# victorramirez952/tomography_3d_reconstructor

Hardware: AMD Instinct MI355X
Metric: Mvoxels/s (SDF+MC) on 1024^3 ellipsoid stack; achieved HBM GB/s vs peak (higher is better)
Workload: dtype f64

## Files before the change

### include/tomo_hip.h

```cpp
#ifndef TOMO_HIP_H
#define TOMO_HIP_H

#include <stddef.h>
#include <stdint.h>

#ifdef __cplusplus
extern "C" {
#endif

#define TOMO_OK 0
#define TOMO_E_ARG (-1)
#define TOMO_E_LAUNCH (-2)
#define TOMO_E_SIZE (-3)
#define TOMO_E_WORKSPACE (-4)

int tomo_abi_version(void);
const char *tomo_error_string(int code);
int tomo_host_mc_cell(const float *h_v, double iso, int8_t *h_tris, int *h_uses_centre);
double tomo_host_mc_edge_offset(double va, double vb);
void tomo_host_mc_centre_offset(const double *h_v8, double *h_out3);

int tomo_host_checksum(const void *h_data, int64_t nbytes, int nthreads, uint64_t *h_out);
int tomo_host_checksum_impl(const void *h_data, int64_t nbytes, int nthreads, int impl, uint64_t *h_out);
int64_t tomo_host_checksum_chunk_bytes(void);
// ... 61 lines not shown
int tomo_field_signs(const float *field, int Nz, int Ny, int Nx, int64_t pitch, int xorg, double iso, int z_begin,
                     int z_end, unsigned long long *signs, uint8_t *gcls, void *stream);

int tomo_mc_classify(const unsigned long long *signs, const uint8_t *gcls, int Nz, int Ny, int Nx, int xorg,
                     unsigned long long *seg_act, uint32_t *seg_cnt, void *stream);
int tomo_mc_scan_segments(const uint32_t *seg_cnt, int64_t nseg, uint32_t *seg_aoff, unsigned long long *totals,
                          void *workspace, int64_t workspace_bytes, void *stream);
int64_t tomo_mc_scan_workspace_bytes(int64_t n);
int tomo_mc_scan(const uint32_t *counts, int64_t n, uint32_t *off_a, uint32_t *off_b, uint32_t *nz_ids,
                 unsigned long long *totals, void *workspace, int64_t workspace_bytes, void *stream);
int tomo_mc_list(int Nz, int Ny, int Nx, int xorg, const uint32_t *seg_aoff, const unsigned long long *seg_act,
                 unsigned long long *vox_key, void *stream);
int tomo_mc_eval(const float *field, int Nz, int Ny, int Nx, int64_t pitch, int xorg, double iso,
                 const unsigned long long *vox_key, int64_t na, uint32_t *vox_counts, uint8_t *vox_flags, void *stream);
int tomo_mc_list_capped(int Nz, int Ny, int Nx, int xorg, const uint32_t *seg_aoff, const unsigned long long *seg_act,
                        unsigned long long *vox_key, int64_t cap, void *stream);
int tomo_mc_eval_capped(const float *field, int Nz, int Ny, int Nx, int64_t pitch, int xorg, double iso,
                        const unsigned long long *vox_key, int64_t cap, const unsigned long long *na_dev,
                        uint32_t *vox_counts, uint8_t *vox_flags, void *stream);
int tomo_mc_emit(const float *field, int Nz, int Ny, int Nx, int64_t pitch, int xorg, double iso,
                 const unsigned long long *vox_key, int64_t na, const unsigned long long *seg_act,
                 const uint32_t *seg_aoff, const uint32_t *vox_voff, const uint32_t *vox_foff, const uint8_t *vox_flags,
                 int z_offset, unsigned long long *vkey, float *vpos, int32_t *faces, unsigned long long *totals,
                 void *stream);

int tomo_mc_first_touch(const float *field, int Nz, int Ny, int Nx, int64_t pitch, int xorg, double iso,
                        const unsigned long long *vox_key, int64_t na, const unsigned long long *seg_act,
                        const uint32_t *seg_aoff, const uint32_t *vox_voff, const uint8_t *vox_flags, int mode,
                        uint32_t *created, const uint32_t *base, int32_t *ft_rank, unsigned long long *totals, void *stream);

int tomo_mc3_list(int Nz, int Ny, int Nx, int xorg, const uint32_t *seg_cnt, const unsigned long long *seg_act,
                  uint32_t *seg_blk, uint32_t *seg_aoff, unsigned long long *vox_key, int64_t cap, unsigned long long *tot,
                  void *stream);
int tomo_mc3_eval(const float *field, int Nz, int Ny, int Nx, int64_t pitch, int xorg, double iso,
                  const unsigned long long *vox_key, int64_t cap, const unsigned long long *tot, int z_offset,
                  uint32_t *vox_loc, int32_t *vox_til, uint8_t *vox_flags, uint16_t *vox_used, float *vox_f3, float *vox_c3,
                  uint32_t *blk3, void *stream);
int64_t tomo_mc3_slice_table_words(int Nz, int Ny);
int64_t tomo_mc3_sort_segments(int Nz, int Ny);
int tomo_mc3_scan(int Nz, int Ny, int Nx, int xorg, const uint32_t *seg_aoff, const uint32_t *vox_loc, int64_t cap,
                  uint32_t *blk3, uint32_t *slice_tab, unsigned long long *tot, int64_t cap_v, int64_t cap_f, void *stream);
int tomo_mc3_vertices(int Nz, int Ny, int Nx, int xorg, const unsigned long long *vox_key, int64_t cap,
                      const unsigned long long *tot, const uint32_t *vox_loc, const uint8_t *vox_flags, const float *vox_f3,
                      const float *vox_c3, const uint32_t *blk3, const uint32_t *slice_tab, int z_offset, int shift,
                      const double *cum, int64_t ncum, const double *adj, int64_t nadj, float mm_y, float mm_x, float *vrec,
                      uint32_t *keys, uint32_t *idx, void *stream);
int64_t tomo_mc3_sort_workspace_bytes(int64_t cap_v, int64_t nseg);
int tomo_mc3_sort_rank_top(const float *vrec, uint32_t *keys, uint32_t *idx, int64_t cap_v, int Nz, int Ny, const uint32_t *slice_tab,
                           unsigned long long *tot, float *uniq, int32_t *table, void *workspace, int64_t workspace_bytes,
                           float z_top, void *stream);
int tomo_mc3_sort_rank_fused(const float *vrec, const uint32_t *keys, int64_t cap_v, int Nz, int Ny, uint32_t *slice_tab,
                             unsigned long long *tot, float *uniq, int32_t *table, float z_top, void *stream);
int tomo_mc3_faces(int Nz, int Ny, int Nx, int xorg, const unsigned long long *vox_key, int64_t cap, unsigned long long *tot,
                   const unsigned long long *seg_act, const uint32_t *seg_aoff, const uint32_t *vox_loc, const int32_t *vox_til,
                   const uint16_t *vox_used, const uint32_t *blk3, const int32_t *table, int64_t *faces, int64_t cap_f,
                   void *stream);

int tomo_vertex_finalize(float *vpos, int64_t nv, int shift, const double *cum, int64_t ncum,
                         const double *adj, int64_t nadj, float mm_y, float mm_x, void *stream);
int64_t tomo_mesh_unique_workspace_bytes(int64_t nv);
int tomo_mesh_unique(const float *vpos, int64_t nv, float *uniq, int32_t *rank, unsigned long long *totals,
                     void *workspace, int64_t workspace_bytes, void *stream);
int tomo_mesh_lookup(const float *uniq, int64_t nu, const float *query, int64_t nq, int32_t *out,
                     unsigned long long *missing, void *stream);
int tomo_slab_top_rows(const float *uniq, const unsigned long long *tot, int64_t cap_v, int64_t cap, float *msg, void *stream);
int tomo_slab_lookup(const float *uniq, const unsigned long long *tot, int64_t cap_v, const float *msg, int64_t cap,
// ... 42 lines not shown
```

### tomography_3d_reconstructor_amd/_lib.py

```python
import ctypes
import os
import subprocess

_HERE = os.path.dirname(os.path.abspath(__file__))
SO_PATH = os.environ.get("TOMO_LIB") or os.path.join(_HERE, "libtomo_hip.so")
CSRC = os.path.join(_HERE, "csrc")

_c_i = ctypes.c_int
_c_i64 = ctypes.c_int64
_c_p = ctypes.c_void_p
_c_d = ctypes.c_double
_c_f = ctypes.c_float

SIGNATURES = {
    "tomo_abi_version": (_c_i, []),
    "tomo_error_string": (ctypes.c_char_p, [_c_i]),
    "tomo_host_mc_cell": (_c_i, [_c_p, _c_d, _c_p, _c_p]),
    "tomo_host_mc_edge_offset": (_c_d, [_c_d, _c_d]),
    "tomo_host_mc_centre_offset": (None, [_c_p, _c_p]),
    "tomo_host_checksum": (_c_i, [_c_p, _c_i64, _c_i, _c_p]),
    "tomo_host_checksum_impl": (_c_i, [_c_p, _c_i64, _c_i, _c_i, _c_p]),
    "tomo_host_checksum_chunk_bytes": (_c_i64, []),
    "tomo_host_checksum_part": (_c_i, [_c_p, _c_i64, _c_i64, _c_i, _c_i, _c_p]),
    "tomo_host_checksum_fold": (_c_i, [_c_p, _c_i64, _c_i64, _c_p]),
# ... 27 lines not shown
    "tomo_pack_close_ends": (_c_i, [_c_p, _c_p, _c_i, _c_i, _c_i, _c_p, _c_p]),
    "tomo_pack_bits_pair": (_c_i, [_c_p, _c_p, _c_i, _c_p, _c_p, _c_i, _c_i, _c_i, _c_p]),
    "tomo_slab_edges": (_c_i, [_c_p, _c_p, _c_i, _c_i, _c_i, _c_i, _c_p, _c_p, _c_i, _c_i, _c_p, _c_p, _c_p, _c_i, _c_p, _c_p, _c_p, _c_p,
                               _c_i, _c_p, _c_p]),
    "tomo_pack_close_range": (_c_i, [_c_p, _c_p, _c_i, _c_i, _c_i, _c_i, _c_i, _c_p, _c_p, _c_i, _c_i, _c_p]),
    "tomo_close_ends_workspace_words": (_c_i64, [_c_i, _c_i, _c_i]),
    "tomo_close_ends_scan": (_c_i, [_c_p, _c_i, _c_i, _c_i, _c_p, _c_p]),
    "tomo_close_ends_gp": (_c_i, [_c_p, _c_i, _c_i, _c_i, _c_p, _c_p, _c_p]),
    "tomo_morph_pass": (_c_i, [_c_p, _c_p, _c_i, _c_i, _c_i, _c_i, _c_p]),
    "tomo_morph_fused": (_c_i, [_c_p, _c_p, _c_i, _c_i, _c_i, ctypes.c_uint32, _c_i, _c_p]),
    "tomo_smooth": (_c_i, [_c_p, _c_p, _c_i, _c_i, _c_i, _c_i, _c_i, _c_p]),
    "tomo_extend_bits": (_c_i, [_c_p, _c_p, _c_i, _c_i, _c_i, _c_i, _c_p]),
    "tomo_field_fill": (_c_i, [_c_p, _c_p, _c_i, _c_i, _c_i, _c_i, _c_i, _c_p, _c_p, _c_p]),
    "tomo_field_fill_bits": (_c_i, [_c_p, _c_p, _c_i, _c_i, _c_i, _c_i, _c_p, _c_p, _c_p]),
    "tomo_field_span_bytes": (_c_i64, [_c_i, _c_i, _c_i, _c_i]),
    "tomo_field_fill_bits_sparse": (_c_i, [_c_p, _c_p, _c_i, _c_i, _c_i, _c_i, _c_p, _c_p, _c_p, _c_p]),
    "tomo_sign_rows": (_c_i64, [_c_i]),
    "tomo_field_signs_fused": (_c_i, [_c_i]),
    "tomo_sign_buffer_words": (_c_i64, [_c_i, _c_i, _c_i, _c_i]),
    "tomo_field_signs": (_c_i, [_c_p, _c_i, _c_i, _c_i, _c_i64, _c_i, _c_d, _c_i, _c_i, _c_p, _c_p, _c_p]),
    "tomo_mc_classify": (_c_i, [_c_p, _c_p, _c_i, _c_i, _c_i, _c_i, _c_p, _c_p, _c_p]),
    "tomo_mc_scan_segments": (_c_i, [_c_p, _c_i64, _c_p, _c_p, _c_p, _c_i64, _c_p]),
    "tomo_mc_scan_workspace_bytes": (_c_i64, [_c_i64]),
    "tomo_mc_scan": (_c_i, [_c_p, _c_i64, _c_p, _c_p, _c_p, _c_p, _c_p, _c_i64, _c_p]),
    "tomo_mc_list": (_c_i, [_c_i, _c_i, _c_i, _c_i, _c_p, _c_p, _c_p, _c_p]),
    "tomo_mc_eval": (_c_i, [_c_p, _c_i, _c_i, _c_i, _c_i64, _c_i, _c_d, _c_p, _c_i64, _c_p, _c_p, _c_p]),
    "tomo_mc_list_capped": (_c_i, [_c_i, _c_i, _c_i, _c_i, _c_p, _c_p, _c_p, _c_i64, _c_p]),
    "tomo_mc_eval_capped": (_c_i, [_c_p, _c_i, _c_i, _c_i, _c_i64, _c_i, _c_d, _c_p, _c_i64, _c_p, _c_p, _c_p, _c_p]),
    "tomo_mc_emit": (_c_i, [_c_p, _c_i, _c_i, _c_i, _c_i64, _c_i, _c_d, _c_p, _c_i64, _c_p, _c_p, _c_p, _c_p, _c_p, _c_i, _c_p,
                            _c_p, _c_p, _c_p, _c_p]),
    "tomo_mc_first_touch": (_c_i, [_c_p, _c_i, _c_i, _c_i, _c_i64, _c_i, _c_d, _c_p, _c_i64, _c_p, _c_p, _c_p, _c_p, _c_i, _c_p,
                                   _c_p, _c_p, _c_p, _c_p]),
    "tomo_mc3_list": (_c_i, [_c_i, _c_i, _c_i, _c_i, _c_p, _c_p, _c_p, _c_p, _c_p, _c_i64, _c_p, _c_p]),
    "tomo_mc3_eval": (_c_i, [_c_p, _c_i, _c_i, _c_i, _c_i64, _c_i, _c_d, _c_p, _c_i64, _c_p, _c_i, _c_p, _c_p, _c_p, _c_p, _c_p,
                             _c_p, _c_p, _c_p]),
    "tomo_mc3_slice_table_words": (_c_i64, [_c_i, _c_i]),
    "tomo_mc3_sort_segments": (_c_i64, [_c_i, _c_i]),
    "tomo_mc3_scan": (_c_i, [_c_i, _c_i, _c_i, _c_i, _c_p, _c_p, _c_i64, _c_p, _c_p, _c_p, _c_i64, _c_i64, _c_p]),
    "tomo_mc3_vertices": (_c_i, [_c_i, _c_i, _c_i, _c_i, _c_p, _c_i64, _c_p, _c_p, _c_p, _c_p, _c_p, _c_p, _c_p, _c_i, _c_i,
                                 _c_p, _c_i64, _c_p, _c_i64, _c_f, _c_f, _c_p, _c_p, _c_p, _c_p]),
    "tomo_mc3_sort_workspace_bytes": (_c_i64, [_c_i64, _c_i64]),
    "tomo_mc3_sort_rank_top": (_c_i, [_c_p, _c_p, _c_p, _c_i64, _c_i, _c_i, _c_p, _c_p, _c_p, _c_p, _c_p, _c_i64, _c_f, _c_p]),
    "tomo_mc3_sort_rank_fused": (_c_i, [_c_p, _c_p, _c_i64, _c_i, _c_i, _c_p, _c_p, _c_p, _c_p, _c_f, _c_p]),
    "tomo_mc3_faces": (_c_i, [_c_i, _c_i, _c_i, _c_i, _c_p, _c_i64, _c_p, _c_p, _c_p, _c_p, _c_p, _c_p, _c_p, _c_p, _c_p, _c_i64, _c_p]),
    "tomo_vertex_finalize": (_c_i, [_c_p, _c_i64, _c_i, _c_p, _c_i64, _c_p, _c_i64, _c_f, _c_f, _c_p]),
    "tomo_mesh_unique_workspace_bytes": (_c_i64, [_c_i64]),
    "tomo_mesh_unique": (_c_i, [_c_p, _c_i64, _c_p, _c_p, _c_p, _c_p, _c_i64, _c_p]),
    "tomo_mesh_lookup": (_c_i, [_c_p, _c_i64, _c_p, _c_i64, _c_p, _c_p, _c_p]),
    "tomo_slab_top_rows": (_c_i, [_c_p, _c_p, _c_i64, _c_i64, _c_p, _c_p]),
    "tomo_slab_lookup": (_c_i, [_c_p, _c_p, _c_i64, _c_p, _c_i64, _c_p, _c_p, _c_p]),
    "tomo_slab_summary": (_c_i, [_c_p, _c_i64, _c_p, _c_p, _c_i64, _c_i64, _c_p, _c_p]),
    "tomo_slab_lookup_summary": (_c_i, [_c_p, _c_p, _c_i64, _c_p, _c_i64, _c_p, _c_i64, _c_i64, _c_p, _c_p, _c_p]),
    "tomo_mc3_faces_slab": (_c_i, [_c_i, _c_i, _c_i, _c_i, _c_p, _c_i64, _c_p, _c_p, _c_p, _c_p, _c_p, _c_p, _c_p, _c_p, _c_p, _c_i64,
                                   _c_p, _c_i, _c_i, _c_p, _c_i64, _c_i64, _c_p]),
    "tomo_mesh_volume_area": (_c_i, [_c_p, _c_p, _c_i64, _c_p, _c_p]),
    "tomo_layer_colors": (_c_i, [_c_p, _c_i, _c_i64, _c_i64, _c_d, _c_d, _c_i, _c_d, _c_d, _c_i, _c_p, _c_p]),
    "tomo_mesh_edge_table_bytes": (_c_i64, [_c_i64]),
    "tomo_mesh_edges": (_c_i, [_c_p, _c_i64, _c_i64, _c_p, _c_i64, _c_p, _c_p]),
    "tomo_mesh_seam_edges": (_c_i, [_c_p, _c_i64, _c_i64, _c_i64, _c_p, _c_i64, _c_p, _c_p]),
    "tomo_mesh_seam_merge": (_c_i, [_c_p, _c_i64, _c_i64, _c_p, _c_i64, _c_p, _c_p]),
    "tomo_mesh_orient_workspace_bytes": (_c_i64, [_c_i64]),
    "tomo_mesh_orient": (_c_i, [_c_p, _c_i64, _c_i64, _c_p, _c_i64, _c_p, _c_p, _c_p]),
    "tomo_mesh_signed_volume": (_c_i, [_c_p, _c_p, _c_i64, _c_p, _c_p, _c_p]),
    "tomo_glb_pack_faces": (_c_i, [_c_p, _c_i64, _c_p, _c_p, _c_p, _c_i, _c_p]),
    "tomo_glb_pack_positions": (_c_i, [_c_p, _c_i, _c_i64, _c_p, _c_p, _c_p]),
    "tomo_mesh_vertex_normals_workspace_bytes": (_c_i64, [_c_i64, _c_i64]),
# ... 49 lines not shown
```

### tomography_3d_reconstructor_amd/csrc/mc.hip

```cpp
#include <cstring>
#include <cstdlib>
#include "tomo_common.h"
#include <rocprim/rocprim.hpp>

#define MC_LUT_QUAL __device__ const
#define MC_FN __device__ static inline
#include "mc_cell.h"

#define SEG 256
#define KEY_XBITS 20
static_assert(KEY_XBITS + 2 == TOMO_KEY_ROW_SHIFT, "key layout shared with mesh.hip");

struct McGrid {
    int Nz, Ny, Nx;
    int64_t pitch;
    int xorg;
    int segs_per_row;
    double iso;
};

typedef float float4u __attribute__((ext_vector_type(4), aligned(4)));
typedef float float2u __attribute__((ext_vector_type(2), aligned(4)));
typedef float float3u __attribute__((ext_vector_type(3), aligned(4)));
typedef int int3u __attribute__((ext_vector_type(3), aligned(4)));
// ... 27 lines not shown
    const int Y = divmod_pos(task, g.Ny, &tz);
    const int s = divmod_pos(tz, g.segs_per_row, &zq);
    const int Z = z_begin + (int)zq;
    const int X0 = s * SEG + lane * 4 - SEG_SHIFT - g.xorg;
    const int64_t NyP = tomo_sign_rows_dev(g.Ny);
    const float *row = field + ((int64_t)Z * g.Ny + Y) * g.pitch + g.xorg;
    float v[4];
#pragma unroll
    for (int k = 0; k < 4; k++) v[k] = (X0 + k >= 0 && X0 + k < g.Nx) ? row[X0 + k] : 0.0f;
    u64 b0 = __ballot((double)v[0] > g.iso), b1 = __ballot((double)v[1] > g.iso);
    u64 b2 = __ballot((double)v[2] > g.iso), b3 = __ballot((double)v[3] > g.iso);
    if (lane < 4)
        signs[((((int64_t)Z * g.segs_per_row + s) * NyP) + Y) * 4 + lane] = lane == 0 ? b0 : (lane == 1 ? b1 : (lane == 2 ? b2 : b3));
}

struct Rec4 { u64 b[4]; };

__device__ static inline Rec4 load_rec(const u64 *__restrict__ signs, int64_t idx)
{
    const ulonglong2 *q = (const ulonglong2 *)(signs + idx * 4);
    ulonglong2 lo = q[0], hi = q[1];
    Rec4 r; r.b[0] = lo.x; r.b[1] = lo.y; r.b[2] = hi.x; r.b[3] = hi.y;
    return r;
}

__device__ static inline Rec4 rec_of(const u64 *__restrict__ signs, int64_t idx, int gc)
{
    if (gc == 2) return load_rec(signs, idx);
    Rec4 r;
    r.b[0] = r.b[1] = r.b[2] = r.b[3] = gc ? ~0ull : 0ull;
    return r;
}

__global__ __launch_bounds__(256) void mc_classify_bits_kernel(const u64 *__restrict__ signs,
                                                               const unsigned char *__restrict__ gcls, const McGrid g,
                                                               int64_t ntasks, u64 *__restrict__ seg_act,
                                                               u32 *__restrict__ seg_cnt)
{
    const int64_t task = (int64_t)blockIdx.x * blockDim.x + threadIdx.x;
    if (task >= ntasks) return;
    int64_t tz, zq;
    const int Y = divmod_pos(task, g.Ny, &tz);
    const int s = divmod_pos(tz, g.segs_per_row, &zq);
    const int Z = (int)zq;
    const int S = g.segs_per_row;
    const int Yn = Y + 1 < g.Ny ? Y + 1 : g.Ny - 1, Z1 = Z + 1 < g.Nz ? Z + 1 : g.Nz - 1;
    const int Xbase = s * SEG - SEG_SHIFT - g.xorg;
    const int64_t segi = ((int64_t)Z * g.Ny + Y) * S + s;
    if (Xbase >= g.Nx || Xbase + SEG <= 0) { seg_cnt[segi] = 0u; return; }
    const bool has_next = s + 1 < S;
    const int64_t NyP = tomo_sign_rows_dev(g.Ny);
    const int64_t ia = ((int64_t)Z * S + s) * NyP + Y, ib = ((int64_t)Z * S + s) * NyP + Yn;
    const int64_t ic = ((int64_t)Z1 * S + s) * NyP + Y, id = ((int64_t)Z1 * S + s) * NyP + Yn;
    const int64_t G = NyP >> 4;
    const int64_t qa = ((int64_t)Z * G + (Y >> 4)) * S + s, qb = ((int64_t)Z * G + (Yn >> 4)) * S + s;
    const int64_t qc = ((int64_t)Z1 * G + (Y >> 4)) * S + s, qd = ((int64_t)Z1 * G + (Yn >> 4)) * S + s;
    const int ga = gcls[qa], gb = gcls[qb], gc = gcls[qc], gd = gcls[qd];
    const int na = has_next ? gcls[qa + 1] : ga, nb = has_next ? gcls[qb + 1] : gb;
    const int nc = has_next ? gcls[qc + 1] : gc, nd = has_next ? gcls[qd + 1] : gd;
    if (ga != 2 && ga == gb && ga == gc && ga == gd && na == ga && nb == ga && nc == ga && nd == ga) {
        seg_cnt[segi] = 0u;
        return;
    }
    Rec4 R[4] = {rec_of(signs, ia, ga), rec_of(signs, ib, gb), rec_of(signs, ic, gc), rec_of(signs, id, gd)};
    u64 nx0[4];
    nx0[0] = has_next ? (na == 2 ? signs[(ia + NyP) * 4] & 1ull : (u64)na) : 0ull;
    nx0[1] = has_next ? (nb == 2 ? signs[(ib + NyP) * 4] & 1ull : (u64)nb) : 0ull;
    nx0[2] = has_next ? (nc == 2 ? signs[(ic + NyP) * 4] & 1ull : (u64)nc) : 0ull;
    nx0[3] = has_next ? (nd == 2 ? signs[(id + NyP) * 4] & 1ull : (u64)nd) : 0ull;
    u64 act[4];
    u64 any_nonzero = 0;
#pragma unroll
    for (int k = 0; k < 4; k++) {
        int lo = Xbase + k < 0 ? (-(Xbase + k) + 3) / 4 : 0;
        int hi = (g.Nx - 1 - Xbase - k) >= 0 ? (g.Nx - 1 - Xbase - k) / 4 : -1;
        if (hi > 63) hi = 63;
        u64 vmask = 0;
        if (hi >= lo) vmask = (hi - lo == 63) ? ~0ull : (((1ull << (hi - lo + 1)) - 1ull) << lo);
        int dl = g.Nx - 1 - Xbase - k;
        u64 lastm = (dl >= 0 && (dl & 3) == 0 && (dl >> 2) < 64) ? (1ull << (dl >> 2)) : 0ull;
        u64 any = 0, all = ~0ull;
#pragma unroll
        for (int r = 0; r < 4; r++) {
            u64 cur = R[r].b[k];
            u64 nxt = k < 3 ? R[r].b[k + 1] : ((R[r].b[0] >> 1) | (nx0[r] << 63));
            nxt = (nxt & ~lastm) | (cur & lastm);
            any |= cur | nxt;
            all &= cur & nxt;
        }
        act[k] = any & ~all & vmask;
        any_nonzero |= act[k];
    }
    seg_cnt[segi] = any_nonzero ? (u32)(__popcll(act[0]) + __popcll(act[1]) + __popcll(act[2]) + __popcll(act[3])) : 0u;
    if (any_nonzero) {
        ulonglong2 *o = (ulonglong2 *)(seg_act + segi * 4);
        o[0] = make_ulonglong2(act[0], act[1]);
        o[1] = make_ulonglong2(act[2], act[3]);
    }
}

static inline int make_grid(McGrid &g, const float *field, int Nz, int Ny, int Nx, int64_t pitch, int xorg, double iso)
{
    if (!field || Nz < 2 || Ny < 2 || Nx < 2 || pitch < Nx + xorg) return TOMO_E_ARG;
    if (Nx >= (1 << KEY_XBITS)) return TOMO_E_SIZE;
    g.Nz = Nz; g.Ny = Ny; g.Nx = Nx; g.pitch = pitch; g.xorg = xorg; g.iso = iso;
    g.segs_per_row = (int)tomo_mc_segments_per_row(Nx, xorg);
    return TOMO_OK;
}

TOMO_API int tomo_field_signs(const float *field, int Nz, int Ny, int Nx, int64_t pitch, int xorg, double iso,
                              int z_begin, int z_end, unsigned long long *signs, uint8_t *gcls, void *stream)
{
    McGrid g;
    int rc = make_grid(g, field, Nz, Ny, Nx, pitch, xorg, iso);
    if (rc) return rc;
    if (!signs || !gcls || z_begin < 0 || z_end > Nz || z_begin > z_end) return TOMO_E_ARG;
    {
        const int64_t per_slice = (tomo_sign_rows(Ny) >> 4) * g.segs_per_row;
        if (z_end > z_begin && hipMemsetAsync(gcls + z_begin * per_slice, 2, (size_t)((z_end - z_begin) * per_slice),
                                              (hipStream_t)stream) != hipSuccess)
            return TOMO_E_LAUNCH;
    }
    int64_t ntasks = (int64_t)(z_end - z_begin) * g.segs_per_row * Ny;
    if (ntasks == 0) return TOMO_OK;
    int64_t blocks = ceil_div64(ntasks, 4);
    if (blocks > 0x7fffffff) return TOMO_E_SIZE;
    hipLaunchKernelGGL(field_signs_kernel, dim3((unsigned)blocks), dim3(256), 0, (hipStream_t)stream, field, g, z_begin,
                       ntasks, (u64 *)signs);
    return tomo_status();
}

TOMO_API int tomo_mc_classify(const unsigned long long *signs, const uint8_t *gcls, int Nz, int Ny, int Nx, int xorg,
                              unsigned long long *seg_act, uint32_t *seg_cnt, void *stream)
{
    if (!signs || !gcls || !seg_act || !seg_cnt || Nz < 2 || Ny < 2 || Nx < 2) return TOMO_E_ARG;
    if (Nx >= (1 << KEY_XBITS)) return TOMO_E_SIZE;
    McGrid g; g.Nz = Nz; g.Ny = Ny; g.Nx = Nx; g.pitch = 0; g.xorg = xorg; g.iso = 0.0;
    g.segs_per_row = (int)tomo_mc_segments_per_row(Nx, xorg);
    int64_t nseg = (int64_t)Nz * Ny * g.segs_per_row;
    int64_t blocks = ceil_div64(nseg, 256);
    if (blocks > 0x7fffffff) return TOMO_E_SIZE;
    hipLaunchKernelGGL(mc_classify_bits_kernel, dim3((unsigned)blocks), dim3(256), 0, (hipStream_t)stream,
                       (const u64 *)signs, gcls, g, nseg, (u64 *)seg_act, seg_cnt);
    return tomo_status();
}

struct ScanPair { u32 a, b; };
struct ScanUnpack {
    __host__ __device__ rocprim::tuple<u32, u32> operator()(u32 c) const { return rocprim::make_tuple(c & 0xffffu, c >> 16); }
};
struct ScanAdd {
    __host__ __device__ rocprim::tuple<u32, u32> operator()(const rocprim::tuple<u32, u32> &x,
                                                            const rocprim::tuple<u32, u32> &y) const
    {
        return rocprim::make_tuple(rocprim::get<0>(x) + rocprim::get<0>(y), rocprim::get<1>(x) + rocprim::get<1>(y));
    }
};

__global__ void scan_finish_kernel(u32 *__restrict__ off_a, u32 *__restrict__ off_b, int64_t n, u64 *__restrict__ totals)
{
    if (threadIdx.x == 0 && blockIdx.x == 0) {
        off_a[0] = 0u;
        if (off_b) off_b[0] = 0u;
        totals[0] = off_a[n];
        totals[1] = off_b ? off_b[n] : 0ull;
        totals[2] = 0ull;
        totals[3] = 0ull;
    }
}

static size_t scan_temp_bytes(int64_t n)
{
    size_t t1 = 0, t2 = 0;
    size_t m = (size_t)(n > 0 ? n : 1);
    (void)rocprim::inclusive_scan(nullptr, t1, (u32 *)nullptr, (u32 *)nullptr, m, rocprim::plus<u32>(), (hipStream_t)0);
    auto in = rocprim::make_transform_iterator((const u32 *)nullptr, ScanUnpack());
// ... 436 lines not shown
                if ((dx | dy | dz) == 0) v = (flags & (1 << slot)) ? vox_voff[i] + (u32)__popc(flags & ((1 << slot) - 1)) : 0xffffffffu;
                else v = find_vertex(make_key(c.row + dy + dz * rowY, ox, 0), slot, g, seg_act, seg_aoff, vox_voff, vox_flags);
                if (v == 0xffffffffu) atomicAdd(&totals[3], 1ull);
                else ft_rank[v] = (int32_t)(base[i] + n);
            }
            n++;
        }
    }
    if (mode == 0) created[i] = n;
}

TOMO_API int tomo_mc_first_touch(const float *field, int Nz, int Ny, int Nx, int64_t pitch, int xorg, double iso,
                                 const unsigned long long *vox_key, int64_t na, const unsigned long long *seg_act,
                                 const uint32_t *seg_aoff, const uint32_t *vox_voff, const uint8_t *vox_flags, int mode,
                                 uint32_t *created,
                                 const uint32_t *base, int32_t *ft_rank, unsigned long long *totals, void *stream)
{
    McGrid g;
    int rc = make_grid(g, field, Nz, Ny, Nx, pitch, xorg, iso);
    if (rc) return rc;
    if (!vox_key || !seg_act || !seg_aoff || !vox_voff || !vox_flags || !totals || (mode == 0 && !created) ||
        (mode == 1 && (!base || !ft_rank)) || (mode != 0 && mode != 1))
        return TOMO_E_ARG;
    if (na <= 0) return TOMO_OK;
    int64_t blocks = ceil_div64(na, 256);
    if (blocks > 0x7fffffff) return TOMO_E_SIZE;
    hipLaunchKernelGGL(mc_first_touch_kernel, dim3((unsigned)blocks), dim3(256), 0, (hipStream_t)stream, field, g,
                       (const u64 *)vox_key, na, (const u64 *)seg_act, seg_aoff, vox_voff, vox_flags, mode, created, base, ft_rank,
                       (u64 *)totals);
    return tomo_status();
}

#define MC3_BLK 256
#define MC3_LOC_A(l) ((l) & 1023u)
#define MC3_LOC_B(l) (((l) >> 10) & 1023u)
#define MC3_LOC_T(l) ((l) >> 20)

__global__ __launch_bounds__(256) void mc3_segsum_kernel(const u32 *__restrict__ seg_cnt, int64_t nseg, u32 *__restrict__ seg_blk,
                                                         int64_t nblk)
{
    const int lane = threadIdx.x & 63;
    const int64_t b = (int64_t)blockIdx.x * 4 + (threadIdx.x >> 6);
    if (b >= nblk) return;
    const int64_t i0 = b * MC3_BLK + lane * 4;
    u32 s = 0;
    if (i0 + 3 < nseg) {
        const uint4 v = *(const uint4 *)(seg_cnt + i0);
        s = v.x + v.y + v.z + v.w;
    } else {
        for (int k = 0; k < 4; k++) if (i0 + k < nseg) s += seg_cnt[i0 + k];
    }
    s = wave_sum(s);
    if (lane == 0) seg_blk[b] = s;
}

template <int K>
__device__ static inline void scan_small_inplace(u32 *__restrict__ a, int64_t stride, int64_t n, u64 *total_out, u32 *lds )
{
    const int lane = threadIdx.x & 63, w = threadIdx.x >> 6;
    u32 carry[K];
    u64 wide[K];
#pragma unroll
    for (int k = 0; k < K; k++) { carry[k] = 0; wide[k] = 0; }
    for (int64_t base = 0; base < n; base += 1024 * 8) {
        const int64_t i0 = base + (int64_t)threadIdx.x * 8;
        u32 v[K][8], s[K];
// ... 72 lines not shown
    const int64_t seg = (int64_t)blockIdx.x * MC3_BLK + threadIdx.x;
    const u32 cnt = seg < nseg ? seg_cnt[seg] : 0u;
    const u32 inc = wave_inclusive_scan(cnt);
    if (lane == 63) wsum[w] = inc;
    __syncthreads();
    u32 o = seg_blk[blockIdx.x] + inc - cnt;
    for (int k = 0; k < w; k++) o += wsum[k];
    if (seg >= nseg) return;
    seg_aoff[seg] = o;
    if (seg == nseg - 1) seg_aoff[nseg] = o + cnt;
    if (cnt == 0) return;
    if ((u64)o + cnt > (u64)cap || tot[0] > (u64)cap) {
        if (o <= cap) atomicOr((unsigned long long *)&tot[3], 1ull);
        return;
    }
    int64_t row;
    const int s = divmod_pos(seg, g.segs_per_row, &row);
    const ulonglong2 *q = (const ulonglong2 *)(seg_act + seg * 4);
    const ulonglong2 lo = q[0], hi = q[1];
    const u64 b0 = lo.x, b1 = lo.y, b2 = hi.x, b3 = hi.y;
    const int Xs = s * SEG - SEG_SHIFT - g.xorg;
    u64 any = b0 | b1 | b2 | b3;
    while (any) {
        const int L = __ffsll((long long)any) - 1;
        any &= any - 1;
        const int X0 = Xs + 4 * L;
        if ((b0 >> L) & 1ull) vox_key[o++] = make_key(row, X0, 0);
        if ((b1 >> L) & 1ull) vox_key[o++] = make_key(row, X0 + 1, 0);
        if ((b2 >> L) & 1ull) vox_key[o++] = make_key(row, X0 + 2, 0);
        if ((b3 >> L) & 1ull) vox_key[o++] = make_key(row, X0 + 3, 0);
    }
}

TOMO_API int tomo_mc3_list(int Nz, int Ny, int Nx, int xorg, const uint32_t *seg_cnt, const unsigned long long *seg_act,
                           uint32_t *seg_blk, uint32_t *seg_aoff, unsigned long long *vox_key, int64_t cap,
                           unsigned long long *tot, void *stream)
{
    if (Nz < 2 || Ny < 2 || Nx < 2 || !seg_cnt || !seg_act || !seg_blk || !seg_aoff || !vox_key || !tot) return TOMO_E_ARG;
    if (cap <= 0 || cap >= 0x1fffffffll) return TOMO_E_SIZE;
    if (Nx >= (1 << KEY_XBITS)) return TOMO_E_SIZE;
    McGrid g; g.Nz = Nz; g.Ny = Ny; g.Nx = Nx; g.pitch = 0; g.xorg = xorg; g.iso = 0.0;
    g.segs_per_row = (int)tomo_mc_segments_per_row(Nx, xorg);
    const int64_t nseg = (int64_t)Nz * Ny * g.segs_per_row, nblk = ceil_div64(nseg, MC3_BLK);
    if (nblk > 0x7fffffff) return TOMO_E_SIZE;
    hipStream_t s = (hipStream_t)stream;
    hipLaunchKernelGGL(mc3_segsum_kernel, dim3((unsigned)ceil_div64(nblk, 4)), dim3(256), 0, s, seg_cnt, nseg, seg_blk, nblk);
    hipLaunchKernelGGL(mc3_scan_seg_kernel, dim3(1), dim3(1024), 0, s, seg_blk, nblk, (u64 *)tot);
    hipLaunchKernelGGL(mc3_list_kernel, dim3((unsigned)nblk), dim3(MC3_BLK), 0, s, g, seg_cnt, (const u32 *)seg_blk,
                       (const u64 *)seg_act, nseg, seg_aoff, (u64 *)vox_key, (u32)cap, (u64 *)tot);
    return tomo_status();
}

__global__ __launch_bounds__(MC3_BLK) void mc3_eval_kernel(const float *__restrict__ field, const McGrid g,
                                                           const u64 *__restrict__ vox_key, int64_t cap,
                                                           const u64 *__restrict__ tot, int z_offset,
                                                           u32 *__restrict__ vox_loc, int32_t *__restrict__ vox_til,
                                                           uint8_t *__restrict__ vox_flags, uint16_t *__restrict__ vox_used,
                                                           float *__restrict__ vox_f3, float *__restrict__ vox_c3,
                                                           u32 *__restrict__ blk3, int64_t nblk)
{
    __shared__ u32 wsum[4];
    const int lane = threadIdx.x & 63, w = threadIdx.x >> 6;
    const int64_t i = (int64_t)blockIdx.x * MC3_BLK + threadIdx.x;
    const u64 na = tot[0];
    const bool live = i < cap && (u64)i < na && na <= (u64)cap;
    u32 packed = 0;
    if (live) {
        Cell c;
        load_cell(field, g, vox_key[i], c);
        int ntri = 0;
        int32_t til = 0;
        u32 used = 0;
        if (c.cell_ok && c.index != 0 && c.index != 255) {
            const McTiling t = mc_cell_tiling(c.v, c.index);
            ntri = t.ntri;
            if (t.centre) c.flags |= 8;
            til = (int32_t)(((intptr_t)t.tris - (intptr_t)LUT_TILING1) * 16 + ntri);
            const int ix = c.index;
#define BICH(a, b) ((u32)(((ix >> (a)) ^ (ix >> (b))) & 1))
            used = BICH(0, 1) | BICH(1, 2) << 1 | BICH(2, 3) << 2 | BICH(3, 0) << 3 | BICH(4, 5) << 4 | BICH(5, 6) << 5 | BICH(6, 7) << 6 |
                   BICH(7, 4) << 7 | BICH(0, 4) << 8 | BICH(1, 5) << 9 | BICH(2, 6) << 10 | BICH(3, 7) << 11 | (t.centre ? 1u << 12 : 0u);
#undef BICH
            if (ntri == 0) used = 0;
// ... 378 lines not shown
```

### tomography_3d_reconstructor_amd/pipeline.py

```python
import math
import os
import threading
from dataclasses import dataclass

import numpy as np
import torch

from . import _lib


COUNTERS = dict.fromkeys(("na_hint_hit", "na_hint_miss", "mc3_hint_hit", "mc3_hint_miss", "mc3_sort_fused", "mc3_sort_library",
                          "mc3_exact", "mc3_general_unique", "mc3_degenerate"), 0)
NA_HINTS = os.environ.get("TOMO_NA_HINTS", "1") not in ("", "0")
_NA_HINT = {}
LIST_LIMIT = 2 ** 31
MESH_LIMIT = 2 ** 31
PACK_CLOSE_FUSED = os.environ.get("TOMO_PACK_CLOSE", "1") not in ("", "0")
FIELD_FROM_BITS = True
FIELD_SPARSE = os.environ.get("TOMO_FIELD_SPARSE", "0") not in ("", "0")


def _stream():
    return torch.cuda.current_stream().cuda_stream

# ... 505 lines not shown

    def __init__(self, t):
        t = t.reshape(-1)
        self._key = (str(t.device), threading.get_ident(), int(t.numel()))
        pool = PendingDownload._free.setdefault(self._key, [])
        self._host = pool.pop() if pool else torch.empty(t.numel(), dtype=torch.int64, pin_memory=True)
        self._host.copy_(t, non_blocking=True)
        self._event = torch.cuda.Event()
        self._event.record(torch.cuda.current_stream(t.device))

    def wait(self, timeout_s=None):
        if timeout_s is None:
            self._event.synchronize()
        else:
            wait_event(self._event, timeout_s, "the counters of a pass")
        out = self._host.tolist()
        PendingDownload._free[self._key].append(self._host)
        self._host = None
        return out


class Mc3Surface:

    def __init__(self, f, slice_depths, mm_per_pixel_y, mm_per_pixel_x, add_padding=True, z_offset=0, z_top=None, tot=None):
        self.field, self.z_offset = f, int(z_offset)
        self.z_top = float("nan") if z_top is None else float(z_top)
        self.hint_key = (f.Nz, f.Ny, f.Nx, self.z_offset)
        self._depth = _depth_args(slice_depths, add_padding, f.data.device)
        self._mm = (float(np.float32(mm_per_pixel_y)), float(np.float32(mm_per_pixel_x)))
        self.tot = torch.empty(8, dtype=torch.int64, device=f.data.device) if tot is None else tot
        self.uniq = self.table = self.faces_final = None
        self.nv = self.nf = self.na = 0
        self.deferred = False
        self._pending = None

    def classify(self):
        L, f, dev = _lib.lib(), self.field, self.field.data.device
        if f.signs is None or f.signs_level != 0.5:
            if f.sparse:
                raise _lib.TomoError("a sparse field holds floats only near the 0.5 surface")
            field_signs(f, 0.5)
        nseg = f.Nz * f.Ny * L.tomo_mc_segments_per_row(f.Nx, f.xorg)
        self.seg_act = torch.empty(nseg * 4, dtype=torch.int64, device=dev)
        self.seg_cnt = torch.empty(nseg, dtype=torch.int32, device=dev)
        _lib.check(L.tomo_mc_classify(_p(f.signs), _p(f.gcls), f.Nz, f.Ny, f.Nx, f.xorg, _p(self.seg_act), _p(self.seg_cnt), _stream()),
                   "tomo_mc_classify")
        self.seg_blk = torch.empty((nseg + 255) // 256, dtype=torch.int32, device=dev)
        self.seg_aoff = torch.empty(nseg + 1, dtype=torch.int32, device=dev)

    def build_list(self, cap):
        f, self.cap = self.field, cap
        self.vox_key = torch.empty(cap, dtype=torch.int64, device=f.data.device)
        _lib.check(_lib.lib().tomo_mc3_list(f.Nz, f.Ny, f.Nx, f.xorg, _p(self.seg_cnt), _p(self.seg_act), _p(self.seg_blk), _p(self.seg_aoff),
                                            _p(self.vox_key), cap, _p(self.tot), _stream()), "tomo_mc3_list")

    def eval_scan(self, cap_v, cap_f):
        L, f, cap, st, dev = _lib.lib(), self.field, self.cap, _stream(), self.field.data.device
        self.vox_loc = torch.empty(cap, dtype=torch.int32, device=dev)
        self.vox_til = torch.empty(cap, dtype=torch.int32, device=dev)
        self.vox_flags = torch.empty(cap, dtype=torch.uint8, device=dev)
        self.vox_used = torch.empty(cap, dtype=torch.int16, device=dev)
        self.vox_f3 = torch.empty(3 * cap, dtype=torch.float32, device=dev)
        self.vox_c3 = torch.empty(3 * cap, dtype=torch.float32, device=dev)
        self.blk3 = torch.empty(3 * ((cap + 255) // 256), dtype=torch.int32, device=dev)
        self.slice_tab = torch.empty(L.tomo_mc3_slice_table_words(f.Nz, f.Ny), dtype=torch.int32, device=dev)
        _lib.check(L.tomo_mc3_eval(_p(f.data), f.Nz, f.Ny, f.Nx, f.pitch, f.xorg, 0.5, _p(self.vox_key), cap, _p(self.tot), self.z_offset,
                                   _p(self.vox_loc), _p(self.vox_til), _p(self.vox_flags), _p(self.vox_used), _p(self.vox_f3),
                                   _p(self.vox_c3), _p(self.blk3), st), "tomo_mc3_eval")
        _lib.check(L.tomo_mc3_scan(f.Nz, f.Ny, f.Nx, f.xorg, _p(self.seg_aoff), _p(self.vox_loc), cap, _p(self.blk3), _p(self.slice_tab),
                                   _p(self.tot), cap_v, cap_f, st), "tomo_mc3_scan")

    def vertices_sort(self, cap_v):
        L, f, cap, tot, st, dev = _lib.lib(), self.field, self.cap, self.tot, _stream(), self.field.data.device
        cum_t, ncum, adj_t, nadj = self._depth
        self.cap_v = cap_v
        self.vrec = torch.empty((cap_v, 4), dtype=torch.float32, device=dev)
        keys = torch.empty(cap_v, dtype=torch.int32, device=dev)
        self.rows = torch.empty((cap_v, 3), dtype=torch.float32, device=dev)
        self.table = torch.empty(4 * cap, dtype=torch.int32, device=dev)
        fused = FUSED_SORT and not _MC3_LARGE.get(self.hint_key)
        idx = None if fused else torch.empty(cap_v, dtype=torch.int32, device=dev)
        _lib.check(L.tomo_mc3_vertices(f.Nz, f.Ny, f.Nx, f.xorg, _p(self.vox_key), cap, _p(tot), _p(self.vox_loc), _p(self.vox_flags),
                                       _p(self.vox_f3), _p(self.vox_c3), _p(self.blk3), _p(self.slice_tab), self.z_offset, 1, _p(cum_t), ncum,
                                       _p(adj_t), nadj, *self._mm, _p(self.vrec), _p(keys), _p(idx), st), "tomo_mc3_vertices")
        if fused:
            COUNTERS["mc3_sort_fused"] += 1
            _lib.check(L.tomo_mc3_sort_rank_fused(_p(self.vrec), _p(keys), cap_v, f.Nz, f.Ny, _p(self.slice_tab), _p(tot), _p(self.rows),
# ... 426 lines not shown
```

Measured before the change: 660,300.

## Fuse per-block segment count sums into the MC3 classify kernel

```diff
diff --git a/include/tomo_hip.h b/include/tomo_hip.h
--- a/include/tomo_hip.h
+++ b/include/tomo_hip.h
@@ -117,6 +117,11 @@
 int tomo_mc3_list(int Nz, int Ny, int Nx, int xorg, const uint32_t *seg_cnt, const unsigned long long *seg_act,
                   uint32_t *seg_blk, uint32_t *seg_aoff, unsigned long long *vox_key, int64_t cap, unsigned long long *tot,
                   void *stream);
+int tomo_mc3_classify(const unsigned long long *signs, const uint8_t *gcls, int Nz, int Ny, int Nx, int xorg,
+                      unsigned long long *seg_act, uint32_t *seg_cnt, uint32_t *seg_blk, void *stream);
+int tomo_mc3_list_summed(int Nz, int Ny, int Nx, int xorg, const uint32_t *seg_cnt, const unsigned long long *seg_act,
+                         uint32_t *seg_blk, uint32_t *seg_aoff, unsigned long long *vox_key, int64_t cap,
+                         unsigned long long *tot, void *stream);
 int tomo_mc3_eval(const float *field, int Nz, int Ny, int Nx, int64_t pitch, int xorg, double iso,
                   const unsigned long long *vox_key, int64_t cap, const unsigned long long *tot, int z_offset,
                   uint32_t *vox_loc, int32_t *vox_til, uint8_t *vox_flags, uint16_t *vox_used, float *vox_f3, float *vox_c3,
diff --git a/tomography_3d_reconstructor_amd/_lib.py b/tomography_3d_reconstructor_amd/_lib.py
--- a/tomography_3d_reconstructor_amd/_lib.py
+++ b/tomography_3d_reconstructor_amd/_lib.py
@@ -83,6 +83,8 @@
     "tomo_mc_first_touch": (_c_i, [_c_p, _c_i, _c_i, _c_i, _c_i64, _c_i, _c_d, _c_p, _c_i64, _c_p, _c_p, _c_p, _c_p, _c_i, _c_p,
                                    _c_p, _c_p, _c_p, _c_p]),
     "tomo_mc3_list": (_c_i, [_c_i, _c_i, _c_i, _c_i, _c_p, _c_p, _c_p, _c_p, _c_p, _c_i64, _c_p, _c_p]),
+    "tomo_mc3_classify": (_c_i, [_c_p, _c_p, _c_i, _c_i, _c_i, _c_i, _c_p, _c_p, _c_p, _c_p]),
+    "tomo_mc3_list_summed": (_c_i, [_c_i, _c_i, _c_i, _c_i, _c_p, _c_p, _c_p, _c_p, _c_p, _c_i64, _c_p, _c_p]),
     "tomo_mc3_eval": (_c_i, [_c_p, _c_i, _c_i, _c_i, _c_i64, _c_i, _c_d, _c_p, _c_i64, _c_p, _c_i, _c_p, _c_p, _c_p, _c_p, _c_p,
                              _c_p, _c_p, _c_p]),
     "tomo_mc3_slice_table_words": (_c_i64, [_c_i, _c_i]),
diff --git a/tomography_3d_reconstructor_amd/csrc/mc.hip b/tomography_3d_reconstructor_amd/csrc/mc.hip
--- a/tomography_3d_reconstructor_amd/csrc/mc.hip
+++ b/tomography_3d_reconstructor_amd/csrc/mc.hip
@@ -83,43 +83,27 @@
     return r;
 }
 
-__global__ __launch_bounds__(256) void mc_classify_bits_kernel(const u64 *__restrict__ signs,
-                                                               const unsigned char *__restrict__ gcls, const McGrid g,
-                                                               int64_t ntasks, u64 *__restrict__ seg_act,
-                                                               u32 *__restrict__ seg_cnt)
-{
-    const int64_t task = (int64_t)blockIdx.x * blockDim.x + threadIdx.x;
-    if (task >= ntasks) return;
-    int64_t tz, zq;
-    const int Y = divmod_pos(task, g.Ny, &tz);
-    const int s = divmod_pos(tz, g.segs_per_row, &zq);
-    const int Z = (int)zq;
+__device__ static inline u32 classify_seg(const u64 *__restrict__ signs, const McGrid &g, int Z, int Y, int s, const int cls[4],
+                                          const int ncls[4], u64 act[4])
+{
     const int S = g.segs_per_row;
+    const int Xbase = s * SEG - SEG_SHIFT - g.xorg;
+    if (Xbase >= g.Nx || Xbase + SEG <= 0) return 0u;
+    const int ga = cls[0], gb = cls[1], gc = cls[2], gd = cls[3];
+    const int na = ncls[0], nb = ncls[1], nc = ncls[2], nd = ncls[3];
+    if (ga != 2 && ga == gb && ga == gc && ga == gd && na == ga && nb == ga && nc == ga && nd == ga)
+        return 0u;
     const int Yn = Y + 1 < g.Ny ? Y + 1 : g.Ny - 1, Z1 = Z + 1 < g.Nz ? Z + 1 : g.Nz - 1;
-    const int Xbase = s * SEG - SEG_SHIFT - g.xorg;
-    const int64_t segi = ((int64_t)Z * g.Ny + Y) * S + s;
-    if (Xbase >= g.Nx || Xbase + SEG <= 0) { seg_cnt[segi] = 0u; return; }
     const bool has_next = s + 1 < S;
     const int64_t NyP = tomo_sign_rows_dev(g.Ny);
     const int64_t ia = ((int64_t)Z * S + s) * NyP + Y, ib = ((int64_t)Z * S + s) * NyP + Yn;
     const int64_t ic = ((int64_t)Z1 * S + s) * NyP + Y, id = ((int64_t)Z1 * S + s) * NyP + Yn;
-    const int64_t G = NyP >> 4;
-    const int64_t qa = ((int64_t)Z * G + (Y >> 4)) * S + s, qb = ((int64_t)Z * G + (Yn >> 4)) * S + s;
-    const int64_t qc = ((int64_t)Z1 * G + (Y >> 4)) * S + s, qd = ((int64_t)Z1 * G + (Yn >> 4)) * S + s;
-    const int ga = gcls[qa], gb = gcls[qb], gc = gcls[qc], gd = gcls[qd];
-    const int na = has_next ? gcls[qa + 1] : ga, nb = has_next ? gcls[qb + 1] : gb;
-    const int nc = has_next ? gcls[qc + 1] : gc, nd = has_next ? gcls[qd + 1] : gd;
-    if (ga != 2 && ga == gb && ga == gc && ga == gd && na == ga && nb == ga && nc == ga && nd == ga) {
-        seg_cnt[segi] = 0u;
-        return;
-    }
     Rec4 R[4] = {rec_of(signs, ia, ga), rec_of(signs, ib, gb), rec_of(signs, ic, gc), rec_of(signs, id, gd)};
     u64 nx0[4];
     nx0[0] = has_next ? (na == 2 ? signs[(ia + NyP) * 4] & 1ull : (u64)na) : 0ull;
     nx0[1] = has_next ? (nb == 2 ? signs[(ib + NyP) * 4] & 1ull : (u64)nb) : 0ull;
     nx0[2] = has_next ? (nc == 2 ? signs[(ic + NyP) * 4] & 1ull : (u64)nc) : 0ull;
     nx0[3] = has_next ? (nd == 2 ? signs[(id + NyP) * 4] & 1ull : (u64)nd) : 0ull;
-    u64 act[4];
     u64 any_nonzero = 0;
 #pragma unroll
     for (int k = 0; k < 4; k++) {
@@ -142,12 +126,91 @@
         act[k] = any & ~all & vmask;
         any_nonzero |= act[k];
     }
-    seg_cnt[segi] = any_nonzero ? (u32)(__popcll(act[0]) + __popcll(act[1]) + __popcll(act[2]) + __popcll(act[3])) : 0u;
-    if (any_nonzero) {
-        ulonglong2 *o = (ulonglong2 *)(seg_act + segi * 4);
-        o[0] = make_ulonglong2(act[0], act[1]);
-        o[1] = make_ulonglong2(act[2], act[3]);
-    }
+    return any_nonzero ? (u32)(__popcll(act[0]) + __popcll(act[1]) + __popcll(act[2]) + __popcll(act[3])) : 0u;
+}
+
+__device__ static inline void store_act(u64 *__restrict__ seg_act, int64_t segi, const u64 act[4])
+{
+    ulonglong2 *o = (ulonglong2 *)(seg_act + segi * 4);
+    o[0] = make_ulonglong2(act[0], act[1]);
+    o[1] = make_ulonglong2(act[2], act[3]);
+}
+
+__global__ __launch_bounds__(256) void mc_classify_bits_kernel(const u64 *__restrict__ signs,
+                                                               const unsigned char *__restrict__ gcls, const McGrid g,
+                                                               int64_t ntasks, u64 *__restrict__ seg_act,
+                                                               u32 *__restrict__ seg_cnt)
+{
+    const int64_t task = (int64_t)blockIdx.x * blockDim.x + threadIdx.x;
+    if (task >= ntasks) return;
+    int64_t tz, zq;
+    const int Y = divmod_pos(task, g.Ny, &tz);
+    const int s = divmod_pos(tz, g.segs_per_row, &zq);
+    const int Z = (int)zq;
+    const int S = g.segs_per_row;
+    const int Yn = Y + 1 < g.Ny ? Y + 1 : g.Ny - 1, Z1 = Z + 1 < g.Nz ? Z + 1 : g.Nz - 1;
+    const int64_t segi = ((int64_t)Z * g.Ny + Y) * S + s;
+    const bool has_next = s + 1 < S;
+    const int64_t G = tomo_sign_rows_dev(g.Ny) >> 4;
+    const int64_t qa = ((int64_t)Z * G + (Y >> 4)) * S + s, qb = ((int64_t)Z * G + (Yn >> 4)) * S + s;
+    const int64_t qc = ((int64_t)Z1 * G + (Y >> 4)) * S + s, qd = ((int64_t)Z1 * G + (Yn >> 4)) * S + s;
+    const int cls[4] = {gcls[qa], gcls[qb], gcls[qc], gcls[qd]};
+    const int ncls[4] = {has_next ? gcls[qa + 1] : cls[0], has_next ? gcls[qb + 1] : cls[1],
+                         has_next ? gcls[qc + 1] : cls[2], has_next ? gcls[qd + 1] : cls[3]};
+    u64 act[4];
+    const u32 cnt = classify_seg(signs, g, Z, Y, s, cls, ncls, act);
+    seg_cnt[segi] = cnt;
+    if (cnt) store_act(seg_act, segi, act);
+}
+
+#define MC3_SEGBLK 256
+__global__ __launch_bounds__(256) void mc3_classify_kernel(const u64 *__restrict__ signs, const unsigned char *__restrict__ gcls,
+                                                           const McGrid g, int64_t nseg, int64_t nblk, u64 *__restrict__ seg_act,
+                                                           u32 *__restrict__ seg_cnt, u32 *__restrict__ seg_blk)
+{
+    const int lane = threadIdx.x & 63;
+    const int64_t b = (int64_t)blockIdx.x * 4 + (threadIdx.x >> 6);
+    if (b >= nblk) return;
+    const int S = g.segs_per_row;
+    const int64_t G = tomo_sign_rows_dev(g.Ny) >> 4;
+    const int64_t i0 = b * MC3_SEGBLK + lane * 4;
+    int64_t row, zq;
+    int s = divmod_pos(i0, S, &row);
+    int Y = divmod_pos(row, g.Ny, &zq);
+    int Z = (int)zq;
+    int cls[4], ncls[4];
+    u32 cnt[4] = {0u, 0u, 0u, 0u};
+    bool fresh = true;
+#pragma unroll
+    for (int j = 0; j < 4; j++) {
+        if (i0 + j >= nseg) break;
+        const int Yn = Y + 1 < g.Ny ? Y + 1 : g.Ny - 1, Z1 = Z + 1 < g.Nz ? Z + 1 : g.Nz - 1;
+        const int64_t q[4] = {((int64_t)Z * G + (Y >> 4)) * S + s, ((int64_t)Z * G + (Yn >> 4)) * S + s,
+                              ((int64_t)Z1 * G + (Y >> 4)) * S + s, ((int64_t)Z1 * G + (Yn >> 4)) * S + s};
+        const bool has_next = s + 1 < S;
+#pragma unroll
+        for (int r = 0; r < 4; r++) {
+            if (fresh) cls[r] = gcls[q[r]];
+            ncls[r] = has_next ? gcls[q[r] + 1] : cls[r];
+        }
+        u64 act[4];
+        cnt[j] = classify_seg(signs, g, Z, Y, s, cls, ncls, act);
+        if (cnt[j]) store_act(seg_act, i0 + j, act);
+        fresh = !has_next;
+#pragma unroll
+        for (int r = 0; r < 4; r++) cls[r] = ncls[r];
+        if (++s == S) {
+            s = 0;
+            if (++Y == g.Ny) { Y = 0; Z++; }
+        }
+    }
+    if (i0 + 3 < nseg && ((uintptr_t)seg_cnt & 15) == 0) {
+        *(uint4 *)(seg_cnt + i0) = make_uint4(cnt[0], cnt[1], cnt[2], cnt[3]);
+    } else {
+        for (int j = 0; j < 4; j++) if (i0 + j < nseg) seg_cnt[i0 + j] = cnt[j];
+    }
+    const u32 sum = wave_sum(cnt[0] + cnt[1] + cnt[2] + cnt[3]);
+    if (lane == 0) seg_blk[b] = sum;
 }
 
 static inline int make_grid(McGrid &g, const float *field, int Nz, int Ny, int Nx, int64_t pitch, int xorg, double iso)
@@ -193,6 +256,20 @@
     if (blocks > 0x7fffffff) return TOMO_E_SIZE;
     hipLaunchKernelGGL(mc_classify_bits_kernel, dim3((unsigned)blocks), dim3(256), 0, (hipStream_t)stream,
                        (const u64 *)signs, gcls, g, nseg, (u64 *)seg_act, seg_cnt);
+    return tomo_status();
+}
+
+TOMO_API int tomo_mc3_classify(const unsigned long long *signs, const uint8_t *gcls, int Nz, int Ny, int Nx, int xorg,
+                               unsigned long long *seg_act, uint32_t *seg_cnt, uint32_t *seg_blk, void *stream)
+{
+    if (!signs || !gcls || !seg_act || !seg_cnt || !seg_blk || Nz < 2 || Ny < 2 || Nx < 2) return TOMO_E_ARG;
+    if (Nx >= (1 << KEY_XBITS)) return TOMO_E_SIZE;
+    McGrid g; g.Nz = Nz; g.Ny = Ny; g.Nx = Nx; g.pitch = 0; g.xorg = xorg; g.iso = 0.0;
+    g.segs_per_row = (int)tomo_mc_segments_per_row(Nx, xorg);
+    const int64_t nseg = (int64_t)Nz * Ny * g.segs_per_row, nblk = ceil_div64(nseg, MC3_SEGBLK);
+    if (nblk > 0x7fffffff) return TOMO_E_SIZE;
+    hipLaunchKernelGGL(mc3_classify_kernel, dim3((unsigned)ceil_div64(nblk, 4)), dim3(256), 0, (hipStream_t)stream,
+                       (const u64 *)signs, gcls, g, nseg, nblk, (u64 *)seg_act, seg_cnt, seg_blk);
     return tomo_status();
 }
 
@@ -695,6 +772,7 @@
 }
 
 #define MC3_BLK 256
+static_assert(MC3_SEGBLK == MC3_BLK, "mc3_classify_kernel sums seg_cnt over the list kernel's blocks");
 #define MC3_LOC_A(l) ((l) & 1023u)
 #define MC3_LOC_B(l) (((l) >> 10) & 1023u)
 #define MC3_LOC_T(l) ((l) >> 20)
@@ -833,9 +911,9 @@
     }
 }
 
-TOMO_API int tomo_mc3_list(int Nz, int Ny, int Nx, int xorg, const uint32_t *seg_cnt, const unsigned long long *seg_act,
+static int mc3_list_launch(int Nz, int Ny, int Nx, int xorg, const uint32_t *seg_cnt, const unsigned long long *seg_act,
                            uint32_t *seg_blk, uint32_t *seg_aoff, unsigned long long *vox_key, int64_t cap,
-                           unsigned long long *tot, void *stream)
+                           unsigned long long *tot, void *stream, bool summed)
 {
     if (Nz < 2 || Ny < 2 || Nx < 2 || !seg_cnt || !seg_act || !seg_blk || !seg_aoff || !vox_key || !tot) return TOMO_E_ARG;
     if (cap <= 0 || cap >= 0x1fffffffll) return TOMO_E_SIZE;
@@ -845,11 +923,26 @@
     const int64_t nseg = (int64_t)Nz * Ny * g.segs_per_row, nblk = ceil_div64(nseg, MC3_BLK);
     if (nblk > 0x7fffffff) return TOMO_E_SIZE;
     hipStream_t s = (hipStream_t)stream;
-    hipLaunchKernelGGL(mc3_segsum_kernel, dim3((unsigned)ceil_div64(nblk, 4)), dim3(256), 0, s, seg_cnt, nseg, seg_blk, nblk);
+    if (!summed)
+        hipLaunchKernelGGL(mc3_segsum_kernel, dim3((unsigned)ceil_div64(nblk, 4)), dim3(256), 0, s, seg_cnt, nseg, seg_blk, nblk);
     hipLaunchKernelGGL(mc3_scan_seg_kernel, dim3(1), dim3(1024), 0, s, seg_blk, nblk, (u64 *)tot);
     hipLaunchKernelGGL(mc3_list_kernel, dim3((unsigned)nblk), dim3(MC3_BLK), 0, s, g, seg_cnt, (const u32 *)seg_blk,
                        (const u64 *)seg_act, nseg, seg_aoff, (u64 *)vox_key, (u32)cap, (u64 *)tot);
     return tomo_status();
+}
+
+TOMO_API int tomo_mc3_list(int Nz, int Ny, int Nx, int xorg, const uint32_t *seg_cnt, const unsigned long long *seg_act,
+                           uint32_t *seg_blk, uint32_t *seg_aoff, unsigned long long *vox_key, int64_t cap,
+                           unsigned long long *tot, void *stream)
+{
+    return mc3_list_launch(Nz, Ny, Nx, xorg, seg_cnt, seg_act, seg_blk, seg_aoff, vox_key, cap, tot, stream, false);
+}
+
+TOMO_API int tomo_mc3_list_summed(int Nz, int Ny, int Nx, int xorg, const uint32_t *seg_cnt, const unsigned long long *seg_act,
+                                  uint32_t *seg_blk, uint32_t *seg_aoff, unsigned long long *vox_key, int64_t cap,
+                                  unsigned long long *tot, void *stream)
+{
+    return mc3_list_launch(Nz, Ny, Nx, xorg, seg_cnt, seg_act, seg_blk, seg_aoff, vox_key, cap, tot, stream, true);
 }
 
 __global__ __launch_bounds__(MC3_BLK) void mc3_eval_kernel(const float *__restrict__ field, const McGrid g,
diff --git a/tomography_3d_reconstructor_amd/pipeline.py b/tomography_3d_reconstructor_amd/pipeline.py
--- a/tomography_3d_reconstructor_amd/pipeline.py
+++ b/tomography_3d_reconstructor_amd/pipeline.py
@@ -561,6 +561,7 @@
         self.uniq = self.table = self.faces_final = None
         self.nv = self.nf = self.na = 0
         self.deferred = False
+        self._summed = False
         self._pending = None
 
     def classify(self):
@@ -572,16 +573,19 @@
         nseg = f.Nz * f.Ny * L.tomo_mc_segments_per_row(f.Nx, f.xorg)
         self.seg_act = torch.empty(nseg * 4, dtype=torch.int64, device=dev)
         self.seg_cnt = torch.empty(nseg, dtype=torch.int32, device=dev)
-        _lib.check(L.tomo_mc_classify(_p(f.signs), _p(f.gcls), f.Nz, f.Ny, f.Nx, f.xorg, _p(self.seg_act), _p(self.seg_cnt), _stream()),
-                   "tomo_mc_classify")
         self.seg_blk = torch.empty((nseg + 255) // 256, dtype=torch.int32, device=dev)
+        _lib.check(L.tomo_mc3_classify(_p(f.signs), _p(f.gcls), f.Nz, f.Ny, f.Nx, f.xorg, _p(self.seg_act), _p(self.seg_cnt), _p(self.seg_blk),
+                                       _stream()), "tomo_mc3_classify")
+        self._summed = True
         self.seg_aoff = torch.empty(nseg + 1, dtype=torch.int32, device=dev)
 
     def build_list(self, cap):
-        f, self.cap = self.field, cap
+        L, f, self.cap = _lib.lib(), self.field, cap
         self.vox_key = torch.empty(cap, dtype=torch.int64, device=f.data.device)
-        _lib.check(_lib.lib().tomo_mc3_list(f.Nz, f.Ny, f.Nx, f.xorg, _p(self.seg_cnt), _p(self.seg_act), _p(self.seg_blk), _p(self.seg_aoff),
-                                            _p(self.vox_key), cap, _p(self.tot), _stream()), "tomo_mc3_list")
+        fn, name = (L.tomo_mc3_list_summed, "tomo_mc3_list_summed") if self._summed else (L.tomo_mc3_list, "tomo_mc3_list")
+        self._summed = False
+        _lib.check(fn(f.Nz, f.Ny, f.Nx, f.xorg, _p(self.seg_cnt), _p(self.seg_act), _p(self.seg_blk), _p(self.seg_aoff),
+                      _p(self.vox_key), cap, _p(self.tot), _stream()), name)
 
     def eval_scan(self, cap_v, cap_f):
         L, f, cap, st, dev = _lib.lib(), self.field, self.cap, _stream(), self.field.data.device
```

New measurement: 655,800. No clear change (-0.7%).
